# uzh-rpg/event_representation_study

Hardware: AMD Instinct MI355X
Metric: events/sec/GPU (OptimizedRep, Gen1 640x480) + 12-rep GWD matrix wall-time (higher is better)
Workload: dtype f64

## Files before the change

event_representation_study_amd/csrc/evrep_bin.hip:

```cpp
#include "evrep_common.h"

namespace evrep {

#ifndef EVREP_BIN_THREADS
#define EVREP_BIN_THREADS 256
#endif
constexpr int kBinThreads = EVREP_BIN_THREADS;
constexpr int kBinWaves = kBinThreads / kWave;

template <typename Op>
__device__ inline int wave_reduce_dpp(int v, int identity, Op op) {
    v = op(v, __builtin_amdgcn_update_dpp(identity, v, 0x111, 0xf, 0xf, false));
    v = op(v, __builtin_amdgcn_update_dpp(identity, v, 0x112, 0xf, 0xf, false));
    v = op(v, __builtin_amdgcn_update_dpp(identity, v, 0x114, 0xf, 0xf, false));
    v = op(v, __builtin_amdgcn_update_dpp(identity, v, 0x118, 0xf, 0xf, false));
    v = op(v, __builtin_amdgcn_update_dpp(identity, v, 0x142, 0xa, 0xf, false));
    v = op(v, __builtin_amdgcn_update_dpp(identity, v, 0x143, 0xc, 0xf, false));
    return __builtin_amdgcn_readlane(v, 63);
}
__device__ inline int wave_min(int v) { return wave_reduce_dpp(v, INT32_MAX, [](int a, int b) { return min(a, b); }); }
__device__ inline int wave_max(int v) { return wave_reduce_dpp(v, INT32_MIN, [](int a, int b) { return max(a, b); }); }
__device__ inline uint32_t wave_or(uint32_t v) { return (uint32_t)wave_reduce_dpp((int)v, 0, [](int a, int b) { return a | b; }); }
__device__ inline int wave_sum(int v) { return wave_reduce_dpp(v, 0, [](int a, int b) { return a + b; }); }

__device__ inline void wave_phase_lds() {
    __builtin_amdgcn_fence(__ATOMIC_RELEASE, "wavefront");
    __builtin_amdgcn_wave_barrier();
    __builtin_amdgcn_fence(__ATOMIC_ACQUIRE, "wavefront");
}

struct BlockStats {
    int32_t tmin, tmax, xmin, xmax, ymin, ymax;
    uint32_t neg_flags, oob_flags, status;
    int32_t n_valid;
    int32_t pad[2];
};
static_assert(sizeof(BlockStats) == 48, "BlockStats");

__device__ inline void stats_identity(BlockStats &s) {
    s.tmin = INT32_MAX; s.tmax = INT32_MIN; s.xmin = INT32_MAX; s.xmax = INT32_MIN; s.ymin = INT32_MAX; s.ymax = INT32_MIN;
    s.neg_flags = 0; s.oob_flags = 0; s.status = 0; s.n_valid = 0; s.pad[0] = 0; s.pad[1] = 0;
}
__device__ inline void stats_merge(BlockStats &a, const BlockStats &b) {
    a.tmin = min(a.tmin, b.tmin); a.tmax = max(a.tmax, b.tmax);
    a.xmin = min(a.xmin, b.xmin); a.xmax = max(a.xmax, b.xmax);
    a.ymin = min(a.ymin, b.ymin); a.ymax = max(a.ymax, b.ymax);
    a.neg_flags |= b.neg_flags; a.oob_flags |= b.oob_flags; a.status |= b.status; a.n_valid += b.n_valid;
}
__device__ inline void stats_wave_reduce(BlockStats &s) {
    s.tmin = wave_min(s.tmin); s.tmax = wave_max(s.tmax);
    s.xmin = wave_min(s.xmin); s.xmax = wave_max(s.xmax);
    s.ymin = wave_min(s.ymin); s.ymax = wave_max(s.ymax);
    s.neg_flags = wave_or(s.neg_flags); s.oob_flags = wave_or(s.oob_flags); s.status = wave_or(s.status);
    s.n_valid = wave_sum(s.n_valid);
}

constexpr int kRegBatch = 8;

__device__ inline bool decode_window_block(int B, int nblk, int &b, int &blk) {
    const int id = blockIdx.x;
    const int per_group = 8 * nblk;
    const int grp = id / per_group, r = id - grp * per_group;
    const int nw = min(8, B - 8 * grp);
    if (nw == 8) {
        b = grp * 8 + (r & 7);
        blk = r >> 3;
        return true;
    }
    if (r >= nw * nblk) return false;
    b = grp * 8 + r / nblk;
    blk = r - (r / nblk) * nblk;
    return true;
}

#ifdef EVREP_TU_CORE
static __global__ __launch_bounds__(kBinThreads) void k_row_hist(const int4 *__restrict__ ev, const int64_t *__restrict__ off,
                                                      int B, int H, int W, int chunk, int nblk,
                                                      uint32_t *__restrict__ table, BlockStats *__restrict__ stats) {
    extern __shared__ uint32_t hist[];
    __shared__ BlockStats wstats[kBinWaves];
    int b, blk;
    if (!decode_window_block(B, nblk, b, blk)) return;
    const int64_t beg = off[b];
    const int64_t n = off[b + 1] - beg;
    const int64_t lo = (int64_t)blk * chunk;
    if (lo >= n) return;
    for (int i = threadIdx.x; i < H; i += kBinThreads) hist[i] = 0;
    __syncthreads();
    const int64_t hi = (lo + chunk < n) ? lo + chunk : n;
    const MdesWindows mw = mdes_windows(n);
    const int64_t HW = (int64_t)H * W;
    BlockStats st;
    stats_identity(st);
    for (int64_t r0 = lo; r0 < hi; r0 += (int64_t)kRegBatch * kBinThreads) {
        int4 e[kRegBatch];
        int tprev[kRegBatch];
#pragma unroll
        for (int i = 0; i < kRegBatch; ++i) {
            const int64_t r = r0 + (int64_t)i * kBinThreads + threadIdx.x;
            e[i] = make_int4(0, 0, INT32_MAX, 0);
            tprev[i] = INT32_MIN;
            if (r < hi) {
                e[i] = ev[beg + r];
                if ((threadIdx.x & 63) == 0 && r > 0) tprev[i] = ev[beg + r - 1].z;
            }
        }
#pragma unroll
        for (int i = 0; i < kRegBatch; ++i) {
            const int up = __shfl_up(e[i].z, 1, 64);
            if ((threadIdx.x & 63) != 0) tprev[i] = up;
        }
#pragma unroll
        for (int i = 0; i < kRegBatch; ++i) {
            const int64_t r = r0 + (int64_t)i * kBinThreads + threadIdx.x;
            if (r < hi) {
                const int64_t key = (int64_t)e[i].x + (int64_t)e[i].y * W;
                const uint32_t memb = mdes_membership(mw, (int32_t)r);
                if (e[i].w == -1) st.neg_flags |= memb;
                if (key >= 0 && key < HW) {
                    atomicAdd(&hist[(uint32_t)key / (uint32_t)W], 1u);
                    ++st.n_valid;
                } else {
                    st.status |= EVREP_ST_OOB;
                    const int cls = e[i].w == 1 ? 1 : (e[i].w == -1 ? 2 : (e[i].w == 0 ? 3 : 0));
                    st.oob_flags |= memb | (cls ? (memb << (7 * cls)) : 0u);
                }
                if (tprev[i] > e[i].z) st.status |= EVREP_ST_UNSORTED;
                st.tmin = min(st.tmin, e[i].z); st.tmax = max(st.tmax, e[i].z);
                st.xmin = min(st.xmin, e[i].x); st.xmax = max(st.xmax, e[i].x);
                st.ymin = min(st.ymin, e[i].y); st.ymax = max(st.ymax, e[i].y);
            }
        }
    }
    stats_wave_reduce(st);
    if ((threadIdx.x & 63) == 0) wstats[threadIdx.x >> 6] = st;
    __syncthreads();
    if (threadIdx.x == 0) {
        BlockStats t = wstats[0];
        for (int w = 1; w < kBinWaves; ++w) stats_merge(t, wstats[w]);
        stats[(size_t)b * nblk + blk] = t;
    }
    uint32_t *dst = table + ((size_t)b * nblk + blk) * H;
    for (int i = threadIdx.x; i < H; i += kBinThreads) dst[i] = hist[i];
}
#endif

#ifdef EVREP_TU_CORE
static __global__ __launch_bounds__(kBinThreads) void k_row_scan(const int64_t *__restrict__ off, int H, int chunk, int nblk,
                                                      uint32_t *__restrict__ table, uint32_t *__restrict__ row_off,
                                                      const BlockStats *__restrict__ stats, WindowMeta *__restrict__ meta) {
    extern __shared__ uint32_t rowtot[];
    __shared__ BlockStats wstats[kBinWaves];
    __shared__ uint32_t tmp[kBinWaves];
    const int b = blockIdx.x;
    const int64_t beg = off[b];
    const int64_t n = off[b + 1] - beg;
    const int nb = (int)((n + chunk - 1) / chunk);
    BlockStats st;
    stats_identity(st);
    for (int blk = threadIdx.x; blk < nb; blk += kBinThreads) stats_merge(st, stats[(size_t)b * nblk + blk]);
    stats_wave_reduce(st);
    if ((threadIdx.x & 63) == 0) wstats[threadIdx.x >> 6] = st;
    for (int r = threadIdx.x; r < H; r += kBinThreads) {
        uint32_t run = 0;
        for (int b0 = 0; b0 < nb; b0 += kRegBatch) {
            uint32_t v[kRegBatch];
#pragma unroll
            for (int i = 0; i < kRegBatch; ++i)
                v[i] = (b0 + i < nb) ? table[((size_t)b * nblk + b0 + i) * H + r] : 0u;
#pragma unroll
            for (int i = 0; i < kRegBatch; ++i)
                if (b0 + i < nb) { table[((size_t)b * nblk + b0 + i) * H + r] = run; run += v[i]; }
        }
        rowtot[r] = run;
    }
    __syncthreads();
    const int per = (H + kBinThreads - 1) / kBinThreads;
    const int r0 = threadIdx.x * per;
    uint32_t local = 0;
    for (int k = 0; k < per; ++k) if (r0 + k < H) local += rowtot[r0 + k];
    uint32_t total;
    uint32_t run = block_exclusive_scan<kBinWaves>(local, tmp, &total);
    for (int k = 0; k < per; ++k)
        if (r0 + k < H) { const uint32_t t = rowtot[r0 + k]; rowtot[r0 + k] = run; run += t; }
    __syncthreads();
    uint32_t *ro = row_off + (size_t)b * (H + 1);
    for (int r = threadIdx.x; r < H; r += kBinThreads) ro[r] = (uint32_t)beg + rowtot[r];
    if (threadIdx.x == 0) {
        ro[H] = (uint32_t)beg + total;
        BlockStats t = wstats[0];
        for (int w = 1; w < kBinWaves; ++w) stats_merge(t, wstats[w]);
        WindowMeta m;
        m.tmin = t.tmin; m.tmax = t.tmax; m.xmin = t.xmin; m.xmax = t.xmax; m.ymin = t.ymin; m.ymax = t.ymax;
        m.neg_flags = t.neg_flags; m.oob_flags = t.oob_flags; m.status = t.status; m.n_valid = t.n_valid;
        if (n <= 0) m.status |= EVREP_ST_EMPTY;
        else if (t.tmin == t.tmax) m.status |= EVREP_ST_FLAT_TIME;
        for (int i = 0; i < 6; ++i) m.pad[i] = 0;
        meta[b] = m;
    }
}
#endif

#ifdef EVREP_TU_CORE
static __global__ __launch_bounds__(kBinThreads) void k_row_scatter(const int4 *__restrict__ ev, const int64_t *__restrict__ off,
                                                         int B, int H, int W, int chunk, int nblk,
                                                         const uint32_t *__restrict__ table,
                                                         const uint32_t *__restrict__ row_off, Rec *__restrict__ sorted1) {
    extern __shared__ uint32_t cnt[];
    int b, blk;
    if (!decode_window_block(B, nblk, b, blk)) return;
    const int64_t beg = off[b];
    const int64_t n = off[b + 1] - beg;
    const int64_t lo = (int64_t)blk * chunk;
    if (lo >= n) return;
    const int64_t hi = (lo + chunk < n) ? lo + chunk : n;
    const int64_t nloc = hi - lo;
    const int lane = threadIdx.x & 63, wave = threadIdx.x >> 6;
    const int64_t wlo = lo + nloc * wave / kBinWaves, whi = lo + nloc * (wave + 1) / kBinWaves;
    const int64_t HW = (int64_t)H * W;
    constexpr int kSuper = kRegBatch * kWave;
    const int nsuper = (int)((whi - wlo + kSuper - 1) / kSuper);
    for (int i = threadIdx.x; i < kBinWaves * H; i += kBinThreads) cnt[i] = 0;
    __syncthreads();
    uint32_t *mycnt = cnt + wave * H;
    int4 e[kRegBatch];
    for (int sb = 0; sb < nsuper; ++sb) {
#pragma unroll
        for (int i = 0; i < kRegBatch; ++i) {
            const int64_t r = wlo + (int64_t)sb * kSuper + i * kWave + lane;
            e[i] = make_int4(-1, -1, 0, 0);
            if (r < whi) e[i] = ev[beg + r];
        }
#pragma unroll
        for (int i = 0; i < kRegBatch; ++i) {
            const int64_t r = wlo + (int64_t)sb * kSuper + i * kWave + lane;
            const int64_t key = (int64_t)e[i].x + (int64_t)e[i].y * W;
            if (r < whi && key >= 0 && key < HW) atomicAdd(&mycnt[(uint32_t)key / (uint32_t)W], 1u);
        }
    }
    __syncthreads();
    for (int row = threadIdx.x; row < H; row += kBinThreads) {
        uint32_t base = row_off[(size_t)b * (H + 1) + row] + table[((size_t)b * nblk + blk) * H + row];
#pragma unroll
        for (int w = 0; w < kBinWaves; ++w) { const uint32_t t = cnt[w * H + row]; cnt[w * H + row] = base; base += t; }
    }
    __syncthreads();
    const int nbits = bits_for(H);
    volatile uint32_t *vcnt = mycnt;
    for (int sb = 0; sb < nsuper; ++sb) {
        if (nsuper > 1) {
#pragma unroll
            for (int i = 0; i < kRegBatch; ++i) {
                const int64_t r = wlo + (int64_t)sb * kSuper + i * kWave + lane;
                e[i] = make_int4(-1, -1, 0, 0);
                if (r < whi) e[i] = ev[beg + r];
            }
        }
#pragma unroll
        for (int i = 0; i < kRegBatch; ++i) {
            const int64_t r0 = wlo + (int64_t)sb * kSuper + i * kWave;
            if (r0 >= whi) break;
            const int64_t r = r0 + lane;
            const int64_t key = (int64_t)e[i].x + (int64_t)e[i].y * W;
            const bool valid = r < whi && key >= 0 && key < HW;
            const uint32_t row = valid ? (uint32_t)key / (uint32_t)W : 0u;
            uint32_t rk; bool last;
            wave_match(row, nbits, valid, lane, rk, last);
            uint32_t pos = 0;
            if (valid) {
                pos = vcnt[row] + rk;
                sorted1[pos] = make_int4((int)key, (int)r, e[i].z, e[i].w);
            }
            __builtin_amdgcn_wave_barrier();
            if (valid && last) vcnt[row] = pos + 1;
            __builtin_amdgcn_wave_barrier();
        }
    }
}
#endif

constexpr int kStageRecs = 2048;
__host__ __device__ inline size_t fused_scatter_lds_bytes(int H) {
    return (size_t)(kBinWaves + 3) * H * sizeof(uint32_t) + (size_t)kStageRecs * sizeof(Rec);
}

#ifdef EVREP_TU_CORE
static __global__ __launch_bounds__(kBinThreads) void k_row_scatter_fused(const int4 *__restrict__ ev, const int64_t *__restrict__ off,
                                                               int B, int H, int W, int chunk, int nblk,
                                                               const uint32_t *__restrict__ table,
                                                               const BlockStats *__restrict__ stats,
                                                               uint32_t *__restrict__ row_off, WindowMeta *__restrict__ meta,
                                                               Rec *__restrict__ sorted1) {
    extern __shared__ __align__(16) unsigned char smem_raw[];
    Rec *stage = reinterpret_cast<Rec *>(smem_raw);
    uint32_t *cnt = reinterpret_cast<uint32_t *>(stage + kStageRecs);
    uint32_t *rowtot = cnt + kBinWaves * H;
    uint32_t *lbase = rowtot + H;
    uint32_t *delta = lbase + H;
    __shared__ BlockStats wstats[kBinWaves];
    __shared__ uint32_t tmp[kBinWaves];
    int b, blk;
    if (!decode_window_block(B, nblk, b, blk)) return;
    const int64_t beg = off[b];
    const int64_t n = off[b + 1] - beg;
    const int64_t lo = (int64_t)blk * chunk;
    if (lo >= n && !(blk == 0)) return;
    const int nb = (int)((n + chunk - 1) / chunk);
    if (n <= 0) {
        uint32_t *ro = row_off + (size_t)b * (H + 1);
        for (int r = threadIdx.x; r <= H; r += kBinThreads) ro[r] = (uint32_t)beg;
        if (threadIdx.x == 0) {
            WindowMeta m;
            m.tmin = INT32_MAX; m.tmax = INT32_MIN; m.xmin = INT32_MAX; m.xmax = INT32_MIN; m.ymin = INT32_MAX; m.ymax = INT32_MIN;
            m.neg_flags = 0; m.oob_flags = 0; m.status = EVREP_ST_EMPTY; m.n_valid = 0;
            for (int i = 0; i < 6; ++i) m.pad[i] = 0;
            meta[b] = m;
        }
        return;
    }
    const int64_t hi = (lo + chunk < n) ? lo + chunk : n;
    const int64_t nloc = hi - lo;
    const int lane = threadIdx.x & 63, wave = threadIdx.x >> 6;
    const int64_t wlo = lo + nloc * wave / kBinWaves, whi = lo + nloc * (wave + 1) / kBinWaves;
    const int64_t HW = (int64_t)H * W;
    for (int i = threadIdx.x; i < kBinWaves * H; i += kBinThreads) cnt[i] = 0;
    __syncthreads();
    uint32_t *mycnt = cnt + wave * H;
    int4 e[kRegBatch];
#pragma unroll
    for (int i = 0; i < kRegBatch; ++i) {
        const int64_t r = wlo + i * kWave + lane;
        e[i] = make_int4(-1, -1, 0, 0);
        if (r < whi) e[i] = ev[beg + r];
    }
#pragma unroll
    for (int i = 0; i < kRegBatch; ++i) {
        const int64_t r = wlo + i * kWave + lane;
        const int64_t key = (int64_t)e[i].x + (int64_t)e[i].y * W;
        if (r < whi && key >= 0 && key < HW) atomicAdd(&mycnt[(uint32_t)key / (uint32_t)W], 1u);
    }
    if (blk == 0) {
        BlockStats st;
        stats_identity(st);
        for (int k = threadIdx.x; k < nb; k += kBinThreads) stats_merge(st, stats[(size_t)b * nblk + k]);
        stats_wave_reduce(st);
        if (lane == 0) wstats[wave] = st;
    }
    __syncthreads();
    for (int r = threadIdx.x; r < H; r += kBinThreads) {
        uint32_t tot = 0, before = 0;
        for (int b0 = 0; b0 < nb; b0 += kRegBatch) {
            uint32_t v[kRegBatch];
#pragma unroll
            for (int i = 0; i < kRegBatch; ++i) v[i] = (b0 + i < nb) ? table[((size_t)b * nblk + b0 + i) * H + r] : 0u;
#pragma unroll
            for (int i = 0; i < kRegBatch; ++i) { tot += v[i]; if (b0 + i < blk) before += v[i]; }
        }
        rowtot[r] = tot;
        delta[r] = before;
        uint32_t own = 0;
#pragma unroll
        for (int w = 0; w < kBinWaves; ++w) own += cnt[w * H + r];
        lbase[r] = own;
    }
    __syncthreads();
    const int per = (H + kBinThreads - 1) / kBinThreads;
    const int r0 = threadIdx.x * per;
    uint32_t loc_t = 0, loc_o = 0;
    for (int k = 0; k < per; ++k) if (r0 + k < H) { loc_t += rowtot[r0 + k]; loc_o += lbase[r0 + k]; }
    uint32_t total_t, total_o;
    uint32_t run_t = block_exclusive_scan<kBinWaves>(loc_t, tmp, &total_t);
    uint32_t run_o = block_exclusive_scan<kBinWaves>(loc_o, tmp, &total_o);
    for (int k = 0; k < per; ++k)
        if (r0 + k < H) {
            const uint32_t t = rowtot[r0 + k]; rowtot[r0 + k] = run_t; run_t += t;
            const uint32_t o = lbase[r0 + k];  lbase[r0 + k] = run_o;  run_o += o;
        }
    __syncthreads();
    for (int r = threadIdx.x; r < H; r += kBinThreads) {
        const uint32_t gstart = (uint32_t)beg + rowtot[r] + delta[r];
        uint32_t base = lbase[r];
        delta[r] = gstart - base;
#pragma unroll
        for (int w = 0; w < kBinWaves; ++w) { const uint32_t t = cnt[w * H + r]; cnt[w * H + r] = base; base += t; }
        if (blk == 0) row_off[(size_t)b * (H + 1) + r] = (uint32_t)beg + rowtot[r];
    }
    if (blk == 0 && threadIdx.x == 0) {
        row_off[(size_t)b * (H + 1) + H] = (uint32_t)beg + total_t;
        BlockStats t = wstats[0];
        for (int w = 1; w < kBinWaves; ++w) stats_merge(t, wstats[w]);
        WindowMeta m;
        m.tmin = t.tmin; m.tmax = t.tmax; m.xmin = t.xmin; m.xmax = t.xmax; m.ymin = t.ymin; m.ymax = t.ymax;
        m.neg_flags = t.neg_flags; m.oob_flags = t.oob_flags; m.status = t.status; m.n_valid = t.n_valid;
        if (t.tmin == t.tmax) m.status |= EVREP_ST_FLAT_TIME;
        for (int i = 0; i < 6; ++i) m.pad[i] = 0;
        meta[b] = m;
    }
    __syncthreads();
    const int nbits = bits_for(H);
    volatile uint32_t *vcnt = mycnt;
#pragma unroll
    for (int i = 0; i < kRegBatch; ++i) {
        const int64_t rr0 = wlo + i * kWave;
        if (rr0 >= whi) break;
        const int64_t r = rr0 + lane;
        const int64_t key = (int64_t)e[i].x + (int64_t)e[i].y * W;
        const bool valid = r < whi && key >= 0 && key < HW;
        const uint32_t row = valid ? (uint32_t)key / (uint32_t)W : 0u;
        uint32_t rk; bool last;
        wave_match(row, nbits, valid, lane, rk, last);
        uint32_t pos = 0;
        if (valid) {
            pos = vcnt[row] + rk;
            stage[pos] = make_int4((int)key, (int)r, e[i].z, e[i].w);
        }
        __builtin_amdgcn_wave_barrier();
        if (valid && last) vcnt[row] = pos + 1;
        __builtin_amdgcn_wave_barrier();
    }
    __syncthreads();
    for (uint32_t t = threadIdx.x; t < total_o; t += kBinThreads) {
        const Rec rec = stage[t];
        const uint32_t row = (uint32_t)rec.x / (uint32_t)W;
        sorted1[delta[row] + t] = rec;
    }
}
#endif

#ifdef EVREP_TU_CORE
static __global__ __launch_bounds__(kWave) void k_col_sort(const Rec *__restrict__ sorted1, const uint32_t *__restrict__ row_off,
                                                   int H, int W, int nchunk, Rec *__restrict__ sorted2,
                                                   uint32_t *__restrict__ chunk_off) {
    extern __shared__ uint32_t cnt[];
    const int b = blockIdx.y, row = blockIdx.x;
    const int lane = threadIdx.x;
    const uint32_t rs = row_off[(size_t)b * (H + 1) + row], re = row_off[(size_t)b * (H + 1) + row + 1];
    const uint32_t n = re - rs;
    uint32_t *co = chunk_off + ((size_t)b * H + row) * (nchunk + 1);
    if (n == 0) {
        for (int c = lane; c <= nchunk; c += kWave) co[c] = rs;
        return;
    }
    constexpr uint32_t kSuper = 4 * kWave;
    const int rowbase = row * W;
    const uint32_t nsuper = (n + kSuper - 1) / kSuper;
    Rec e[4];
    for (int i = lane; i < W; i += kWave) cnt[i] = 0;
    __syncthreads();
    for (uint32_t sb = 0; sb < nsuper; ++sb) {
#pragma unroll
        for (int i = 0; i < 4; ++i) {
            const uint32_t j = sb * kSuper + i * kWave + lane;
            e[i] = make_int4(0, 0, 0, 0);
            if (j < n) e[i] = sorted1[rs + j];
        }
#pragma unroll
        for (int i = 0; i < 4; ++i)
            if (sb * kSuper + i * kWave + lane < n) atomicAdd(&cnt[e[i].x - rowbase], 1u);
    }
    __syncthreads();
    const int per = (W + kWave - 1) / kWave;
    const int c0 = lane * per;
    uint32_t local = 0;
    for (int k = 0; k < per; ++k) if (c0 + k < W) local += cnt[c0 + k];
    uint32_t incl = local;
#pragma unroll
    for (int d = 1; d < 64; d <<= 1) { const uint32_t o = __shfl_up(incl, d, 64); if (lane >= d) incl += o; }
    uint32_t run = incl - local;
    for (int k = 0; k < per; ++k)
        if (c0 + k < W) { const uint32_t t = cnt[c0 + k]; cnt[c0 + k] = run; run += t; }
    __syncthreads();
    for (int c = lane; c <= nchunk; c += kWave) co[c] = (c * kChunkPx < W) ? rs + cnt[c * kChunkPx] : re;
    __syncthreads();
    const int nbits = bits_for(W);
    volatile uint32_t *vcnt = cnt;
    for (uint32_t sb = 0; sb < nsuper; ++sb) {
        if (nsuper > 1) {
#pragma unroll
            for (int i = 0; i < 4; ++i) {
                const uint32_t j = sb * kSuper + i * kWave + lane;
                e[i] = make_int4(0, 0, 0, 0);
                if (j < n) e[i] = sorted1[rs + j];
            }
        }
#pragma unroll
        for (int i = 0; i < 4; ++i) {
            const uint32_t j0 = sb * kSuper + i * kWave;
            if (j0 >= n) break;
            const bool valid = j0 + lane < n;
            const uint32_t col = valid ? (uint32_t)(e[i].x - rowbase) : 0u;
            uint32_t rk; bool last;
            wave_match(col, nbits, valid, lane, rk, last);
            uint32_t pos = 0;
            if (valid) {
                pos = vcnt[col] + rk;
                sorted2[rs + pos] = e[i];
            }
            __builtin_amdgcn_wave_barrier();
            if (valid && last) vcnt[col] = pos + 1;
            __builtin_amdgcn_wave_barrier();
        }
    }
}
#endif

#ifndef BS_DEBUG
#define BS_DEBUG 0
#endif
constexpr int kBsThreads = 1024;
constexpr int kBsWaves = kBsThreads / kWave;
constexpr int kBsPerLane = 8;
constexpr int kBsChunk = kBsThreads * kBsPerLane;
constexpr int kBsMaxBlocks = 64;
constexpr int kBsChainBlocks = 16;

__host__ __device__ inline int bs_hp(int H) { return (H + 1) & ~1; }
__host__ __device__ inline size_t block_rowsort_lds_bytes(int H) {
    return (size_t)kBsChunk * sizeof(Rec) + (size_t)kBsWaves * bs_hp(H) * sizeof(uint16_t) + (size_t)(H + 2) * sizeof(uint32_t);
}

#ifdef EVREP_TU_CORE
static __global__ __launch_bounds__(kBsThreads) void k_block_rowsort(const int4 *__restrict__ ev, const int64_t *__restrict__ off,
                                                             int B, int H, int W, int nblk, uint32_t *__restrict__ table,
                                                             BlockStats *__restrict__ stats, Rec *__restrict__ sorted1) {
    extern __shared__ __align__(16) unsigned char smem_raw[];
    Rec *stage = reinterpret_cast<Rec *>(smem_raw);
    const int Hp = bs_hp(H), Hw = Hp >> 1;
    uint16_t *cnt16 = reinterpret_cast<uint16_t *>(stage + kBsChunk);
    uint32_t *cnt32 = reinterpret_cast<uint32_t *>(cnt16);
    uint32_t *lbase = reinterpret_cast<uint32_t *>(cnt16 + (size_t)kBsWaves * Hp);
    __shared__ BlockStats wstats[kBsWaves];
    __shared__ uint32_t tmp[kBsWaves];
    int b, blk;
    if (!decode_window_block(B, nblk, b, blk)) return;
    const int64_t beg = off[b];
    const int64_t n = off[b + 1] - beg;
    const int64_t lo = (int64_t)blk * kBsChunk;
    if (lo >= n) return;
    const int64_t hi = (lo + kBsChunk < n) ? lo + kBsChunk : n;
    const int lane = threadIdx.x & 63, wave = threadIdx.x >> 6;
    const int64_t wlo = lo + (int64_t)wave * (kBsPerLane * kWave);
    const int64_t whi = (wlo + kBsPerLane * kWave < hi) ? wlo + kBsPerLane * kWave : hi;
    const int64_t HW = (int64_t)H * W;
    int4 e[kBsPerLane];
    int tprev[kBsPerLane];
#pragma unroll
    for (int i = 0; i < kBsPerLane; ++i) {
        const int64_t r = wlo + i * kWave + lane;
        e[i] = make_int4(-1, -1, INT32_MAX, 0);
        tprev[i] = INT32_MIN;
        if (r < whi) {
            e[i] = ev[beg + r];
            if (lane == 0 && r > 0) tprev[i] = ev[beg + r - 1].z;
        }
    }
    for (int i = threadIdx.x; i < kBsWaves * Hw; i += kBsThreads) cnt32[i] = 0;
    __syncthreads();
    const MdesWindows mw = mdes_windows(n);
    uint32_t full = 0, part = 0;
#pragma unroll
    for (int i = 0; i < 7; ++i) {
        if (mw.lo[i] <= lo && hi <= mw.hi[i]) full |= 1u << i;
        else if (!(hi <= mw.lo[i] || lo >= mw.hi[i])) part |= 1u << i;
    }
    uint32_t *mycnt32 = cnt32 + wave * Hw;
    BlockStats st;
    stats_identity(st);
    uint32_t rows[kBsPerLane];
    uint32_t sneg = 0;
    bool cut = false;
    if (part) {
        const int32_t a0 = (int32_t)wlo, a1 = (int32_t)whi;
#pragma unroll
        for (int q = 0; q < 7; ++q) cut |= (mw.lo[q] > a0 && mw.lo[q] < a1) || (mw.hi[q] > a0 && mw.hi[q] < a1);
    }
    const uint32_t memb_u = cut ? 0u : (full | (part ? (mdes_membership(mw, (int32_t)wlo) & part) : 0u));
#pragma unroll
    for (int i = 0; i < kBsPerLane; ++i) {
        const int64_t r0 = wlo + i * kWave;
        const int64_t r = r0 + lane;
        const bool in = r < whi;
        const int up = __builtin_amdgcn_update_dpp(0, e[i].z, 0x138 , 0xf, 0xf, false);
        if (lane != 0) tprev[i] = up;

        uint32_t row = (uint32_t)e[i].y;
        bool valid = in && (uint32_t)e[i].x < (uint32_t)W && (uint32_t)e[i].y < (uint32_t)H;
        if (__any(in && (uint32_t)e[i].x >= (uint32_t)W)) {
            const int64_t key = (int64_t)e[i].x + (int64_t)e[i].y * W;
            valid = in && key >= 0 && key < HW;
            if (valid) row = (uint32_t)key / (uint32_t)W;
        }
        rows[i] = valid ? row : 0xffffffffu;
        if (valid && !(BS_DEBUG & 8)) atomicAdd(&mycnt32[row >> 1], 1u << ((row & 1u) * 16));
        if (!(BS_DEBUG & 1)) {
            if (!cut) {
                if (__any(in && e[i].w == -1)) sneg |= memb_u;
            } else if (in && e[i].w == -1) {
                st.neg_flags |= full | (mdes_membership(mw, (int32_t)r) & part);
            }
            if (__any(in && !valid)) {
                if (in && !valid) {
                    const uint32_t memb = cut ? (full | (mdes_membership(mw, (int32_t)r) & part)) : memb_u;
                    st.status |= EVREP_ST_OOB;
                    const int cls = e[i].w == 1 ? 1 : (e[i].w == -1 ? 2 : (e[i].w == 0 ? 3 : 0));
                    st.oob_flags |= memb | (cls ? (memb << (7 * cls)) : 0u);
                }
            }
        }
        if (in && !(BS_DEBUG & 1)) {
            if (valid) ++st.n_valid;
            if (tprev[i] > e[i].z) st.status |= EVREP_ST_UNSORTED;
            if ((uint32_t)(e[i].w + 1) > 2u) st.status |= kStEscaped;
            st.tmin = min(st.tmin, e[i].z); st.tmax = max(st.tmax, e[i].z);
            st.xmin = min(st.xmin, e[i].x); st.xmax = max(st.xmax, e[i].x);
            st.ymin = min(st.ymin, e[i].y); st.ymax = max(st.ymax, e[i].y);
        }
    }
    st.neg_flags |= sneg;
    stats_wave_reduce(st);
    if (lane == 0) wstats[wave] = st;
    __syncthreads();
    uint32_t run = 0;
    if ((int)threadIdx.x < Hw) {
#pragma unroll
        for (int w = 0; w < kBsWaves; ++w) { const uint32_t c = cnt32[w * Hw + threadIdx.x]; cnt32[w * Hw + threadIdx.x] = run; run += c; }
    }
    const uint32_t own0 = run & 0xffffu, own1 = run >> 16;
    uint32_t total;
    const uint32_t ex = block_exclusive_scan<kBsWaves>(own0 + own1, tmp, &total);
    if ((int)threadIdx.x < Hw) {
        const uint32_t l0 = ex, l1 = ex + own0;
        const uint32_t add = l0 | (l1 << 16);
#pragma unroll
        for (int w = 0; w < kBsWaves; ++w) cnt32[w * Hw + threadIdx.x] += add;
        uint32_t *tb = table + ((size_t)b * nblk + blk) * (H + 1);
        const int r0 = 2 * (int)threadIdx.x;
        tb[r0] = l0; lbase[r0] = l0;
        if (r0 + 1 < H) { tb[r0 + 1] = l1; lbase[r0 + 1] = l1; }
    }
    if (threadIdx.x == 0) {
        table[((size_t)b * nblk + blk) * (H + 1) + H] = total;
        BlockStats t = wstats[0];
        for (int w = 1; w < kBsWaves; ++w) stats_merge(t, wstats[w]);
        stats[(size_t)b * nblk + blk] = t;
    }
    __syncthreads();
    const int nbits = bits_for(H);
    volatile uint16_t *vpos = cnt16 + (size_t)wave * Hp;
#pragma unroll
    for (int i = 0; i < kBsPerLane; ++i) {
        if (wlo + i * kWave >= whi) break;
        const bool valid = rows[i] != 0xffffffffu;
        const uint32_t row = valid ? rows[i] : 0u;
        uint32_t rk = 0; bool last = false;
        if (!(BS_DEBUG & 2)) wave_match(row, nbits, valid, lane, rk, last);
        uint32_t pos = 0;
        if (valid) {
            pos = (BS_DEBUG & 2) ? (uint32_t)(wave * 512 + i * 64 + lane) : (uint32_t)vpos[row] + rk;
            const int64_t r = wlo + i * kWave + lane;
            const Rec rec = make_int4((int)((int64_t)e[i].x + (int64_t)e[i].y * W), (int)r, e[i].z, e[i].w);
            if (BS_DEBUG & 16) sorted1[beg + lo + pos] = rec; else stage[pos] = rec;
        }
        __builtin_amdgcn_wave_barrier();
        if (valid && last) vpos[row] = (uint16_t)(pos + 1);
        __builtin_amdgcn_wave_barrier();
    }
    __syncthreads();
    Rec *dst = sorted1 + beg + lo;
    if (!(BS_DEBUG & (4 | 16)))
        for (uint32_t t = threadIdx.x; t < total; t += kBsThreads) dst[t] = stage[t];
}
#endif

#ifndef EVREP_CS_WAVES
#define EVREP_CS_WAVES 8
#endif
constexpr int kCsWaves = EVREP_CS_WAVES;
constexpr int kCsRowWaves = 4;
constexpr int kCsMaxRuns = 128;
__host__ __device__ inline int col_sort_per4(int W) { return ((W + kWave - 1) / kWave + 3) / 4; }
__host__ __device__ inline int col_sort_words(int W) { return kWave * 4 * col_sort_per4(W); }
__host__ __device__ inline int col_sort_wave_words(int W) { return col_sort_words(W) + 2 * kCsMaxRuns; }

#ifndef CS_WAVES
#define CS_WAVES 8
#endif
#ifdef EVREP_TU_CORE
static __global__ __launch_bounds__(kCsWaves * kWave) __attribute__((amdgpu_waves_per_eu(CS_WAVES))) void k_col_sort_runs(const int4 *__restrict__ ev, const Rec *__restrict__ sorted1, const int64_t *__restrict__ off,
                                                                     const uint32_t *__restrict__ table,
                                                                     const BlockStats *__restrict__ stats, int H, int W, int nblk,
                                                                     int nchunk, int kpr, int chunk_shift, int by_key,
                                                                     Rec *__restrict__ sorted2,
                                                                     uint32_t *__restrict__ chunk_off, WindowMeta *__restrict__ meta) {
    extern __shared__ __align__(16) uint32_t cnt_all[];
    const int lane = threadIdx.x & 63, wave = threadIdx.x >> 6;
    const int b = blockIdx.y, unit = blockIdx.x * (int)(blockDim.x >> 6) + wave;
    if (unit >= (by_key ? H * kpr : H)) return;
    const int row = by_key ? unit / kpr : unit;
    const int ck = by_key ? unit - row * kpr : 0;
    const int Wu = by_key ? min(kChunkPx, W - ck * kChunkPx) : W;
    uint32_t *cnt = cnt_all + (size_t)wave * col_sort_wave_words(by_key ? kChunkPx : W);
    const int64_t beg = off[b];
    const int64_t n_win = off[b + 1] - beg;
    const int nb = min((int)(((uint32_t)n_win + (1u << chunk_shift) - 1u) >> chunk_shift), nblk);
    uint32_t ta[2] = {0u, 0u}, tb[2] = {0u, 0u};
#pragma unroll
    for (int h = 0; h < 2; ++h) {
        const int k = lane + h * kWave;
        if (k < nb) {
            const uint32_t *tk = table + ((size_t)b * nblk + k) * ((size_t)H * kpr + 1);
            ta[h] = tk[by_key ? (size_t)unit : (size_t)row * kpr];
            tb[h] = tk[by_key ? (size_t)unit + 1 : (size_t)(row + 1) * kpr];
        }
    }
    if (unit == 0) {
        BlockStats st;
        stats_identity(st);
#pragma unroll
        for (int h = 0; h < 2; ++h) {
            const int k = lane + h * kWave;
            if (k < nb) {
                const int4 *sp = reinterpret_cast<const int4 *>(stats + (size_t)b * nblk + k);
                const int4 q0 = sp[0], q1 = sp[1], q2 = sp[2];
                st.tmin = min(st.tmin, q0.x); st.tmax = max(st.tmax, q0.y); st.xmin = min(st.xmin, q0.z); st.xmax = max(st.xmax, q0.w);
                st.ymin = min(st.ymin, q1.x); st.ymax = max(st.ymax, q1.y);
                st.neg_flags |= (uint32_t)q1.z; st.oob_flags |= (uint32_t)q1.w;
                st.status |= (uint32_t)q2.x; st.n_valid += q2.y;
            }
        }
        stats_wave_reduce(st);
        if (lane == 0) {
            WindowMeta m;
            m.tmin = st.tmin; m.tmax = st.tmax; m.xmin = st.xmin; m.xmax = st.xmax; m.ymin = st.ymin; m.ymax = st.ymax;
            m.neg_flags = st.neg_flags; m.oob_flags = st.oob_flags; m.status = st.status & 0xffffu; m.n_valid = st.n_valid;
            if (n_win <= 0) m.status |= EVREP_ST_EMPTY;
            else if (st.tmin == st.tmax) m.status |= EVREP_ST_FLAT_TIME;
            for (int i = 0; i < 6; ++i) m.pad[i] = 0;
            meta[b] = m;
        }
    }
    constexpr uint32_t kSuper = 4 * kWave;
    const uint32_t rbeg = (uint32_t)beg + (uint32_t)wave_sum((int)(ta[0] + ta[1]));
    const uint32_t len0 = tb[0] - ta[0], len1 = tb[1] - ta[1];
    uint32_t incl0 = len0, incl1 = len1;
#pragma unroll
    for (int d = 1; d < 64; d <<= 1) {
        const uint32_t o0 = __shfl_up(incl0, d, 64), o1 = __shfl_up(incl1, d, 64);
        if (lane >= d) { incl0 += o0; incl1 += o1; }
    }
    const uint32_t tot0 = (uint32_t)__builtin_amdgcn_readlane((int)incl0, 63);
    incl1 += tot0;
    const uint32_t n = (uint32_t)__builtin_amdgcn_readlane((int)incl1, 63);
    const uint32_t pre0 = incl0 - len0, pre1 = incl1 - len1;
    const uint32_t src0 = (uint32_t)beg + ((uint32_t)lane << chunk_shift) + ta[0] - pre0;
    const uint32_t src1 = (uint32_t)beg + ((uint32_t)(lane + kWave) << chunk_shift) + ta[1] - pre1;
    const uint32_t rend = rbeg + n;
    uint32_t *runs = cnt + col_sort_words(by_key ? kChunkPx : W);
    if (nb > kBsChainBlocks) {
        runs[lane] = pre0;
        runs[kWave + lane] = pre1;
        runs[kCsMaxRuns + lane] = src0;
        runs[kCsMaxRuns + kWave + lane] = src1;
        wave_phase_lds();
    }
    const Rec8 *sorted8 = reinterpret_cast<const Rec8 *>(sorted1);
    const int4 *evw = ev + beg;
    auto load = [&](uint32_t at) -> Rec {
        return by_key ? rec8_unpack(sorted8[at], row * W, ck * kChunkPx, evw) : sorted1[at];
    };
    auto fetch = [&](uint32_t j) -> Rec {
        if (nb <= kBsChainBlocks) {
            uint32_t s = (uint32_t)__builtin_amdgcn_readlane((int)src0, 0);
            uint32_t prev = s;
            for (int k = 1; k < nb; ++k) {
                const uint32_t pk = (uint32_t)__builtin_amdgcn_readlane((int)pre0, k);
                const uint32_t sk = (uint32_t)__builtin_amdgcn_readlane((int)src0, k);
                s += (j >= pk) ? sk - prev : 0u;
                prev = sk;
            }
            return load(s + j);
        }
        uint32_t lo = 0, hi = (uint32_t)nb;
#pragma unroll
        for (int step = 0; step < 7; ++step) {
            const uint32_t mid = (lo + hi) >> 1;
            const bool go = hi - lo > 1 && runs[mid] <= j;
            if (hi - lo > 1) { if (go) lo = mid; else hi = mid; }
        }
        return load(runs[kCsMaxRuns + lo] + j);
    };
    Rec e[4];
#pragma unroll
    for (int i = 0; i < 4; ++i) {
        const uint32_t j = i * kWave + lane;
        e[i] = make_int4(0, 0, 0, 0);
        if (j < n) e[i] = fetch(j);
    }
    const int nbits = bits_for(Wu);
    const int per4 = col_sort_per4(Wu);
    uint4 *cnt4 = reinterpret_cast<uint4 *>(cnt) + (size_t)lane * per4;
    volatile uint32_t *vcnt = cnt;
    uint32_t *co = chunk_off + ((size_t)b * H + row) * (nchunk + 1);
    if (by_key && lane == 0) {
        co[ck] = rbeg;
        if (ck == kpr - 1) co[kpr] = rend;
    }
    if (n == 0) {
        if (!by_key) for (int c = lane; c <= nchunk; c += kWave) co[c] = rbeg;
        return;
    }
    const int rowbase = row * W + ck * kChunkPx;
    const uint32_t nsuper = (n + kSuper - 1) / kSuper;
    for (int k = 0; k < per4; ++k) cnt4[k] = make_uint4(0u, 0u, 0u, 0u);
    wave_phase_lds();
#pragma unroll
    for (int i = 0; i < 4; ++i)
        if ((uint32_t)(i * kWave + lane) < n) atomicAdd(&cnt[e[i].x - rowbase], 1u);
    for (uint32_t sb = 1; sb < nsuper; ++sb)
        for (int i = 0; i < 4; ++i) {
            const uint32_t j = sb * kSuper + i * kWave + lane;
            if (j < n) atomicAdd(&cnt[fetch(j).x - rowbase], 1u);
        }
    wave_phase_lds();
    uint32_t local = 0;
    for (int k = 0; k < per4; ++k) { const uint4 v = cnt4[k]; local += v.x + v.y + v.z + v.w; }
    uint32_t inc2 = local;
#pragma unroll
    for (int d = 1; d < 64; d <<= 1) { const uint32_t o = __shfl_up(inc2, d, 64); if (lane >= d) inc2 += o; }
    uint32_t run = inc2 - local;
    for (int k = 0; k < per4; ++k) {
        const uint4 v = cnt4[k];
        uint4 o;
        o.x = run; o.y = o.x + v.x; o.z = o.y + v.y; o.w = o.z + v.z;
        run = o.w + v.w;
        cnt4[k] = o;
    }
    wave_phase_lds();
    if (!by_key) for (int c = lane; c <= nchunk; c += kWave) co[c] = (c * kChunkPx < W) ? rbeg + cnt[c * kChunkPx] : rend;
    wave_phase_lds();
    for (uint32_t sb = 0; sb < nsuper; ++sb) {
#pragma unroll
        for (int i = 0; i < 4; ++i) {
            const uint32_t j0 = sb * kSuper + i * kWave;
            if (j0 >= n) break;
            const bool valid = j0 + lane < n;
            Rec rec = e[i];
            if (sb > 0) { rec = make_int4(0, 0, 0, 0); if (valid) rec = fetch(j0 + lane); }
            const uint32_t col = valid ? (uint32_t)(rec.x - rowbase) : 0u;
            uint32_t rk; bool last;
            wave_match(col, nbits, valid, lane, rk, last);
            uint32_t pos = 0;
            if (valid) {
                pos = vcnt[col] + rk;
                sorted2[rbeg + pos] = rec;
            }
            __builtin_amdgcn_wave_barrier();
            if (valid && last) vcnt[col] = pos + 1;
            __builtin_amdgcn_wave_barrier();
        }
    }
}
#endif

#ifndef KS_DIRECT_WRITE
#define KS_DIRECT_WRITE 0
#endif
#ifndef KS_DEBUG
#define KS_DEBUG 0
#endif
constexpr int kKsHotGroup = 16;
__host__ __device__ inline size_t block_keysort_lds_bytes(int NK, int cap, int chunk) {
    return (size_t)cap * sizeof(Rec8) + (size_t)chunk * sizeof(uint16_t) + (size_t)(NK + 4) * sizeof(uint32_t);
}

#ifndef KS_WAVES_512
#define KS_WAVES_512 6
#endif
#ifndef KS_WAVES_1024
#define KS_WAVES_1024 8
#endif
template <int TPB, int PL = 8>
__global__ __launch_bounds__(TPB) __attribute__((amdgpu_waves_per_eu(TPB == 1024 ? KS_WAVES_1024 : KS_WAVES_512))) void k_block_keysort(const int4 *__restrict__ ev, const int64_t *__restrict__ off,
                                                             int B, int H, int W, int kpr, int nblk, int cap,
                                                             uint32_t *__restrict__ table, BlockStats *__restrict__ stats,
                                                             Rec *__restrict__ sorted1, int64_t *__restrict__ nwin,
                                                             uint32_t *__restrict__ hot) {
    extern __shared__ __align__(16) unsigned char smem_raw[];
    constexpr int kChunk = TPB * PL, kNW = TPB / kWave, kPerWave = PL * kWave;
    if (blockIdx.x == 0 && threadIdx.x < 128) hot[threadIdx.x * 16] = 0u;
    const int NK = H * kpr;
    Rec8 *stage = reinterpret_cast<Rec8 *>(smem_raw);
    uint16_t *rankbuf = reinterpret_cast<uint16_t *>(stage + cap);
    uint32_t *base = reinterpret_cast<uint32_t *>(rankbuf + kChunk);
    __shared__ int bstats[12];
    __shared__ uint32_t tmp[kNW];
    __shared__ uint32_t nhot_s;
    int b, blk;
    if (!decode_window_block(B, nblk, b, blk)) return;
    const int64_t beg = off[b];
    const int64_t n = off[b + 1] - beg;
    const int64_t lo = (int64_t)blk * kChunk;
    if (blk == 0 && threadIdx.x == 0) nwin[b] = n;
    if (lo >= n) return;
    const int nblock = (int)((lo + kChunk < n) ? kChunk : n - lo);
    const int lane = threadIdx.x & 63, wave = threadIdx.x >> 6;
    const int w0 = wave * kPerWave;
    const int lo32 = (int)lo;
    const int4 *evb = ev + beg + lo;
    int4 e[PL];
    int tprev[PL];
#pragma unroll
    for (int i = 0; i < PL; ++i) {
        const int li = w0 + i * kWave + lane;
        e[i] = make_int4(-1, -1, INT32_MAX, 0);
        tprev[i] = INT32_MIN;
        if (li < nblock) {
            e[i] = evb[li];
            if (lane == 0 && (li > 0 || lo > 0)) tprev[i] = evb[li - 1].z;
        }
    }
    for (int i = threadIdx.x; i <= NK; i += TPB) base[i] = 0;
    if (threadIdx.x == 0) nhot_s = 0u;
    if (threadIdx.x < 12) {
        const int f = threadIdx.x;
        bstats[f] = (f == 0 || f == 2 || f == 4) ? INT32_MAX : ((f == 1 || f == 3 || f == 5) ? INT32_MIN : 0);
    }
    __syncthreads();
    const MdesWindows mw = mdes_windows(n);
    uint32_t full = 0, part = 0;
#pragma unroll
    for (int i = 0; i < 7; ++i) {
        if (mw.lo[i] <= lo32 && lo32 + nblock <= mw.hi[i]) full |= 1u << i;
        else if (!(lo32 + nblock <= mw.lo[i] || lo32 >= mw.hi[i])) part |= 1u << i;
    }
    BlockStats st;
    stats_identity(st);
    uint32_t ko[PL];
    uint32_t sneg = 0;
    bool cut = false;
    const int a0 = lo32 + w0, a1 = min(lo32 + w0 + kPerWave, lo32 + nblock);
    if (part) {
#pragma unroll
        for (int q = 0; q < 7; ++q) cut |= (mw.lo[q] > a0 && mw.lo[q] < a1) || (mw.hi[q] > a0 && mw.hi[q] < a1);
    }
    const uint32_t memb_u = cut ? 0u : (full | (part ? (mdes_membership(mw, a0) & part) : 0u));
    const int HW = H * W;
#pragma unroll
    for (int i = 0; i < PL; ++i) {
        const int li = w0 + i * kWave + lane;
        const bool in = li < nblock;
        const int up = __builtin_amdgcn_update_dpp(0, e[i].z, 0x138 , 0xf, 0xf, false);
        if (lane != 0) tprev[i] = up;
        uint32_t row = (uint32_t)e[i].y, col = (uint32_t)e[i].x;
        bool valid = in && (uint32_t)e[i].x < (uint32_t)W && (uint32_t)e[i].y < (uint32_t)H;
        if (__any(in && (uint32_t)e[i].x >= (uint32_t)W)) {
            const int64_t key = (int64_t)e[i].x + (int64_t)e[i].y * W;
            valid = in && key >= 0 && key < (int64_t)HW;
            if (valid) { row = (uint32_t)key / (uint32_t)W; col = (uint32_t)key - row * (uint32_t)W; }
        }
        ko[i] = 0xffffffffu;
        if (valid) {
            const uint32_t key = row * (uint32_t)kpr + (col >> 7);
            ko[i] = key | (atomicAdd(&base[key], 1u) << 16);
        }
        if (KS_DEBUG & 4) continue;
        if (!cut) {
            if (__any(in && e[i].w == -1)) sneg |= memb_u;
        } else if (in && e[i].w == -1) {
            st.neg_flags |= full | (mdes_membership(mw, lo32 + li) & part);
        }
        if (__any(in && !valid)) {
            if (in && !valid) {
                const uint32_t memb = cut ? (full | (mdes_membership(mw, lo32 + li) & part)) : memb_u;
                st.status |= EVREP_ST_OOB;
                const int cls = e[i].w == 1 ? 1 : (e[i].w == -1 ? 2 : (e[i].w == 0 ? 3 : 0));
                st.oob_flags |= memb | (cls ? (memb << (7 * cls)) : 0u);
            }
        }
        if (in) {
            if (valid) ++st.n_valid;
            if (tprev[i] > e[i].z) st.status |= EVREP_ST_UNSORTED;
            if ((uint32_t)(e[i].w + 1) > 2u) st.status |= kStEscaped;
            st.tmin = min(st.tmin, e[i].z); st.tmax = max(st.tmax, e[i].z);
            st.xmin = min(st.xmin, e[i].x); st.xmax = max(st.xmax, e[i].x);
            st.ymin = min(st.ymin, e[i].y); st.ymax = max(st.ymax, e[i].y);
        }
    }
    st.neg_flags |= sneg;
    stats_wave_reduce(st);
    if (lane == 0) {
        atomicMin(&bstats[0], st.tmin); atomicMax(&bstats[1], st.tmax);
        atomicMin(&bstats[2], st.xmin); atomicMax(&bstats[3], st.xmax);
        atomicMin(&bstats[4], st.ymin); atomicMax(&bstats[5], st.ymax);
        atomicOr(reinterpret_cast<uint32_t *>(&bstats[6]), st.neg_flags);
        atomicOr(reinterpret_cast<uint32_t *>(&bstats[7]), st.oob_flags);
        atomicOr(reinterpret_cast<uint32_t *>(&bstats[8]), st.status);
        atomicAdd(&bstats[9], st.n_valid);
    }
    __syncthreads();
    const int per = (NK + TPB - 1) / TPB;
    const int k0 = (int)threadIdx.x * per;
    uint32_t local = 0;
    for (int k = 0; k < per; ++k) if (k0 + k < NK) local += base[k0 + k];
    uint32_t total;
    uint32_t run = block_exclusive_scan<kNW>(local, tmp, &total);
    for (int k = 0; k < per; ++k)
        if (k0 + k < NK) {
            const uint32_t c = base[k0 + k];
            uint32_t tag = 0u;
            if (c > (uint32_t)kKsHotGroup) tag = (atomicAdd(&nhot_s, 1u) + 1u) << 16;
            base[k0 + k] = run | tag;
            run += c;
        }
    if (threadIdx.x == 0) base[NK] = total;
    if (threadIdx.x < 12) reinterpret_cast<int *>(stats + (size_t)b * nblk + blk)[threadIdx.x] = bstats[threadIdx.x];
    __syncthreads();
    uint32_t *tb = table + ((size_t)b * nblk + blk) * ((size_t)NK + 1);
    if (!(KS_DEBUG & 8))
        for (int k = threadIdx.x; k <= NK; k += TPB) tb[k] = base[k] & 0xffffu;
    const uint32_t nhot = nhot_s;
    const uint32_t mine0 = (uint32_t)(w0 + lane);
#pragma unroll
    for (int i = 0; i < PL; ++i) {
        if (ko[i] != 0xffffffffu) {
            const uint32_t bw = base[ko[i] & 0xffffu];
            if (!(bw >> 16)) rankbuf[(bw & 0xffffu) + (ko[i] >> 16)] = (uint16_t)(mine0 + i * kWave);
        }
    }
    if (nhot) {
        constexpr int kHs = kChunk / 16;
        uint32_t *hcnt = reinterpret_cast<uint32_t *>(stage);
        for (uint32_t t = lane; t < nhot; t += kWave) hcnt[wave * kHs + t] = 0u;
        wave_phase_lds();
#pragma unroll
        for (int i = 0; i < PL; ++i)
            if (ko[i] != 0xffffffffu) {
                const uint32_t hsl = base[ko[i] & 0xffffu] >> 16;
                if (hsl) atomicAdd(&hcnt[wave * kHs + hsl - 1u], 1u);
            }
        __syncthreads();
        if (threadIdx.x < nhot) {
            uint32_t acc = 0;
            for (int w = 0; w < kNW; ++w) { const uint32_t c = hcnt[w * kHs + threadIdx.x]; hcnt[w * kHs + threadIdx.x] = acc; acc += c; }
        }
        __syncthreads();
        const int hbits = bits_for((int)nhot);
        volatile uint32_t *vh = hcnt + wave * kHs;
#pragma unroll
        for (int i = 0; i < PL; ++i) {
            const uint32_t bw = ko[i] != 0xffffffffu ? base[ko[i] & 0xffffu] : 0u;
            const bool hot = (bw >> 16) != 0u;
            if (!__any(hot)) continue;
            const uint32_t slot = hot ? (bw >> 16) - 1u : 0u;
            uint32_t rk; bool last;
            wave_match(slot, hbits, hot, lane, rk, last);
            uint32_t pos = 0;
            if (hot) {
                pos = vh[slot] + rk;
                ko[i] = ((bw & 0xffffu) + pos) | 0x80000000u;
            }
            __builtin_amdgcn_wave_barrier();
            if (hot && last) vh[slot] = pos + 1;
            __builtin_amdgcn_wave_barrier();
        }
    }
    __syncthreads();
    {
        uint32_t gb[PL], g[PL], sm[PL];
        uint32_t gmax = 0;
#pragma unroll
        for (int i = 0; i < PL; ++i) {
            gb[i] = 0; g[i] = 0; sm[i] = 0;
            if (ko[i] != 0xffffffffu && !(ko[i] >> 31)) {
                const uint32_t key = ko[i] & 0xffffu;
                const uint32_t bw = base[key];
                gb[i] = bw & 0xffffu;
                g[i] = (bw >> 16) ? 0u : (base[key + 1] & 0xffffu) - gb[i];
                if (KS_DEBUG & 1) { sm[i] = ko[i] >> 16; g[i] = 0; }
                if (g[i] == 1) g[i] = 0;
                gmax = max(gmax, g[i]);
            }
        }
        gmax = (uint32_t)wave_max((int)gmax);
        for (uint32_t j = 0; j < gmax; ++j) {
#pragma unroll
            for (int i = 0; i < PL; ++i)
                if (j < g[i]) sm[i] += (uint32_t)rankbuf[gb[i] + j] < mine0 + (uint32_t)(i * kWave) ? 1u : 0u;
        }
#pragma unroll
        for (int i = 0; i < PL; ++i)
            if (ko[i] != 0xffffffffu) ko[i] = (ko[i] >> 31) ? (ko[i] & 0x7fffffffu) : gb[i] + sm[i];
    }
    if (nhot) __syncthreads();
    Rec8 *dst = reinterpret_cast<Rec8 *>(sorted1) + beg + lo;
#if KS_DIRECT_WRITE
#pragma unroll
    for (int i = 0; i < PL; ++i) {
        if (ko[i] != 0xffffffffu && !(KS_DEBUG & 2)) {
            int col = e[i].x;
            if ((uint32_t)col >= (uint32_t)W) { const uint32_t key = (uint32_t)(e[i].x + e[i].y * W); col = (int)(key % (uint32_t)W); }
            dst[ko[i]] = rec8_pack(col, lo32 + w0 + i * kWave + lane, e[i].z, e[i].w);
        }
    }
    return;
#endif
    for (uint32_t pb = 0; pb < total && !(KS_DEBUG & 2); pb += (uint32_t)cap) {
        if (pb) __syncthreads();
#pragma unroll
        for (int i = 0; i < PL; ++i) {
            const uint32_t pos = ko[i] - pb;
            if (pos < (uint32_t)cap) {
                int col = e[i].x;
                if ((uint32_t)col >= (uint32_t)W) { const uint32_t key = (uint32_t)(e[i].x + e[i].y * W); col = (int)(key % (uint32_t)W); }
                stage[pos] = rec8_pack(col, lo32 + w0 + i * kWave + lane, e[i].z, e[i].w);
            }
        }
        __syncthreads();
        const uint32_t cnt = min((uint32_t)cap, total - pb);
        for (uint32_t t = threadIdx.x; t < cnt; t += TPB) dst[pb + t] = stage[t];
    }
}

#ifdef EVREP_TU_CORE
static __global__ __launch_bounds__(kWave) void k_window_meta(const int64_t *__restrict__ nwin, const BlockStats *__restrict__ stats,
                                                      int nblk, int chunk_shift, WindowMeta *__restrict__ meta) {
    const int b = blockIdx.x, lane = threadIdx.x;
    const int64_t n_win = nwin[b];
    const int nb = min((int)(((uint32_t)n_win + (1u << chunk_shift) - 1u) >> chunk_shift), nblk);
    BlockStats st;
    stats_identity(st);
    for (int k = lane; k < nb; k += kWave) stats_merge(st, stats[(size_t)b * nblk + k]);
    stats_wave_reduce(st);
    if (lane == 0) {
        WindowMeta m;
        m.tmin = st.tmin; m.tmax = st.tmax; m.xmin = st.xmin; m.xmax = st.xmax; m.ymin = st.ymin; m.ymax = st.ymax;
        m.neg_flags = st.neg_flags; m.oob_flags = st.oob_flags; m.status = st.status & 0xffffu; m.n_valid = st.n_valid;
        if (n_win <= 0) m.status |= EVREP_ST_EMPTY;
        else if (st.tmin == st.tmax) m.status |= EVREP_ST_FLAT_TIME;
        for (int i = 0; i < 6; ++i) m.pad[i] = 0;
        meta[b] = m;
    }
}
#endif

}
```

Baseline: 9.215 billion.

## Restructure key-sort binning: defer stats, clamp loads, vectorize writeback and scan

Loads events with clamped indices and carries a single previous timestamp per wave instead of one per slot. The per-event stats and membership work moves into a lambda that, for small PL, runs after the scatter/writeback, taking it off the path to the first barrier. Other changes: the LDS histogram is zeroed with 16-byte stores, the block scan becomes an inline shuffle scan, the wrap check is hoisted into one wave vote, and the staged output is written as paired 16-byte stores. This adds code complexity and register pressure, and the deferred stats add another barrier at the end.

```diff
diff --git a/event_representation_study_amd/csrc/evrep_bin.hip b/event_representation_study_amd/csrc/evrep_bin.hip
--- a/event_representation_study_amd/csrc/evrep_bin.hip
+++ b/event_representation_study_amd/csrc/evrep_bin.hip
@@ -908,52 +908,104 @@
     const int lo32 = (int)lo;
     const int4 *evb = ev + beg + lo;
     int4 e[PL];
-    int tprev[PL];
-#pragma unroll
-    for (int i = 0; i < PL; ++i) {
-        const int li = w0 + i * kWave + lane;
-        e[i] = make_int4(-1, -1, INT32_MAX, 0);
-        tprev[i] = INT32_MIN;
-        if (li < nblock) {
-            e[i] = evb[li];
-            if (lane == 0 && (li > 0 || lo > 0)) tprev[i] = evb[li - 1].z;
-        }
-    }
-    for (int i = threadIdx.x; i <= NK; i += TPB) base[i] = 0;
+#pragma unroll
+    for (int i = 0; i < PL; ++i) e[i] = evb[min(w0 + i * kWave + lane, nblock - 1)];
+    const bool has_prev = w0 < nblock && (w0 > 0 || lo > 0);
+    int tprev0 = evb[has_prev ? w0 - 1 : 0].z;
+    if (!has_prev) tprev0 = INT32_MIN;
+#pragma unroll
+    for (int i = 0; i < PL; ++i)
+        if (w0 + i * kWave + lane >= nblock) e[i] = make_int4(-1, -1, INT32_MAX, 0);
+    for (int i = threadIdx.x; i <= NK / 4; i += TPB) reinterpret_cast<uint4 *>(base)[i] = make_uint4(0u, 0u, 0u, 0u);
     if (threadIdx.x == 0) nhot_s = 0u;
     if (threadIdx.x < 12) {
         const int f = threadIdx.x;
         bstats[f] = (f == 0 || f == 2 || f == 4) ? INT32_MAX : ((f == 1 || f == 3 || f == 5) ? INT32_MIN : 0);
     }
     __syncthreads();
-    const MdesWindows mw = mdes_windows(n);
-    uint32_t full = 0, part = 0;
-#pragma unroll
-    for (int i = 0; i < 7; ++i) {
-        if (mw.lo[i] <= lo32 && lo32 + nblock <= mw.hi[i]) full |= 1u << i;
-        else if (!(lo32 + nblock <= mw.lo[i] || lo32 >= mw.hi[i])) part |= 1u << i;
-    }
-    BlockStats st;
-    stats_identity(st);
+    constexpr bool kStatsLast = PL <= 4;
     uint32_t ko[PL];
-    uint32_t sneg = 0;
-    bool cut = false;
-    const int a0 = lo32 + w0, a1 = min(lo32 + w0 + kPerWave, lo32 + nblock);
-    if (part) {
-#pragma unroll
-        for (int q = 0; q < 7; ++q) cut |= (mw.lo[q] > a0 && mw.lo[q] < a1) || (mw.hi[q] > a0 && mw.hi[q] < a1);
-    }
-    const uint32_t memb_u = cut ? 0u : (full | (part ? (mdes_membership(mw, a0) & part) : 0u));
+    uint32_t vmask = 0;
+    auto block_stats = [&]() {
+        BlockStats st;
+        stats_identity(st);
+        if (!(KS_DEBUG & 4)) {
+            const MdesWindows mw = mdes_windows(n);
+            uint32_t full = 0, part = 0;
+#pragma unroll
+            for (int i = 0; i < 7; ++i) {
+                if (mw.lo[i] <= lo32 && lo32 + nblock <= mw.hi[i]) full |= 1u << i;
+                else if (!(lo32 + nblock <= mw.lo[i] || lo32 >= mw.hi[i])) part |= 1u << i;
+            }
+            bool cut = false;
+            const int a0 = lo32 + w0, a1 = min(lo32 + w0 + kPerWave, lo32 + nblock);
+            if (part) {
+#pragma unroll
+                for (int q = 0; q < 7; ++q) cut |= (mw.lo[q] > a0 && mw.lo[q] < a1) || (mw.hi[q] > a0 && mw.hi[q] < a1);
+            }
+            const uint32_t memb_u = cut ? 0u : (full | (part ? (mdes_membership(mw, a0) & part) : 0u));
+            bool neg = false, oob = false;
+#pragma unroll
+            for (int i = 0; i < PL; ++i) {
+                const int li = w0 + i * kWave + lane;
+                const bool in = li < nblock, valid = (vmask >> i) & 1u;
+                int tprev = __builtin_amdgcn_update_dpp(0, e[i].z, 0x138 , 0xf, 0xf, false);
+                if (lane == 0) tprev = i == 0 ? tprev0 : __builtin_amdgcn_readlane(e[i > 0 ? i - 1 : 0].z, 63);
+                neg |= in && e[i].w == -1;
+                oob |= in && !valid;
+                if (in) {
+                    if (valid) ++st.n_valid;
+                    if (tprev > e[i].z) st.status |= EVREP_ST_UNSORTED;
+                    if ((uint32_t)(e[i].w + 1) > 2u) st.status |= kStEscaped;
+                    st.tmin = min(st.tmin, e[i].z); st.tmax = max(st.tmax, e[i].z);
+                    st.xmin = min(st.xmin, e[i].x); st.xmax = max(st.xmax, e[i].x);
+                    st.ymin = min(st.ymin, e[i].y); st.ymax = max(st.ymax, e[i].y);
+                }
+            }
+            if (!cut) {
+                if (__any(neg)) st.neg_flags |= memb_u;
+            } else if (neg) {
+#pragma unroll
+                for (int i = 0; i < PL; ++i) {
+                    const int li = w0 + i * kWave + lane;
+                    if (li < nblock && e[i].w == -1) st.neg_flags |= full | (mdes_membership(mw, lo32 + li) & part);
+                }
+            }
+            if (__any(oob)) {
+#pragma unroll
+                for (int i = 0; i < PL; ++i) {
+                    const int li = w0 + i * kWave + lane;
+                    if (li < nblock && !((vmask >> i) & 1u)) {
+                        const uint32_t memb = cut ? (full | (mdes_membership(mw, lo32 + li) & part)) : memb_u;
+                        st.status |= EVREP_ST_OOB;
+                        const int cls = e[i].w == 1 ? 1 : (e[i].w == -1 ? 2 : (e[i].w == 0 ? 3 : 0));
+                        st.oob_flags |= memb | (cls ? (memb << (7 * cls)) : 0u);
+                    }
+                }
+            }
+        }
+        stats_wave_reduce(st);
+        if (lane == 0) {
+            atomicMin(&bstats[0], st.tmin); atomicMax(&bstats[1], st.tmax);
+            atomicMin(&bstats[2], st.xmin); atomicMax(&bstats[3], st.xmax);
+            atomicMin(&bstats[4], st.ymin); atomicMax(&bstats[5], st.ymax);
+            atomicOr(reinterpret_cast<uint32_t *>(&bstats[6]), st.neg_flags);
+            atomicOr(reinterpret_cast<uint32_t *>(&bstats[7]), st.oob_flags);
+            atomicOr(reinterpret_cast<uint32_t *>(&bstats[8]), st.status);
+            atomicAdd(&bstats[9], st.n_valid);
+        }
+    };
     const int HW = H * W;
+    bool wraps = false;
+#pragma unroll
+    for (int i = 0; i < PL; ++i) wraps |= w0 + i * kWave + lane < nblock && (uint32_t)e[i].x >= (uint32_t)W;
+    const bool any_wrap = __any(wraps);
 #pragma unroll
     for (int i = 0; i < PL; ++i) {
-        const int li = w0 + i * kWave + lane;
-        const bool in = li < nblock;
-        const int up = __builtin_amdgcn_update_dpp(0, e[i].z, 0x138 , 0xf, 0xf, false);
-        if (lane != 0) tprev[i] = up;
+        const bool in = w0 + i * kWave + lane < nblock;
         uint32_t row = (uint32_t)e[i].y, col = (uint32_t)e[i].x;
         bool valid = in && (uint32_t)e[i].x < (uint32_t)W && (uint32_t)e[i].y < (uint32_t)H;
-        if (__any(in && (uint32_t)e[i].x >= (uint32_t)W)) {
+        if (any_wrap) {
             const int64_t key = (int64_t)e[i].x + (int64_t)e[i].y * W;
             valid = in && key >= 0 && key < (int64_t)HW;
             if (valid) { row = (uint32_t)key / (uint32_t)W; col = (uint32_t)key - row * (uint32_t)W; }
@@ -962,48 +1014,27 @@
         if (valid) {
             const uint32_t key = row * (uint32_t)kpr + (col >> 7);
             ko[i] = key | (atomicAdd(&base[key], 1u) << 16);
-        }
-        if (KS_DEBUG & 4) continue;
-        if (!cut) {
-            if (__any(in && e[i].w == -1)) sneg |= memb_u;
-        } else if (in && e[i].w == -1) {
-            st.neg_flags |= full | (mdes_membership(mw, lo32 + li) & part);
-        }
-        if (__any(in && !valid)) {
-            if (in && !valid) {
-                const uint32_t memb = cut ? (full | (mdes_membership(mw, lo32 + li) & part)) : memb_u;
-                st.status |= EVREP_ST_OOB;
-                const int cls = e[i].w == 1 ? 1 : (e[i].w == -1 ? 2 : (e[i].w == 0 ? 3 : 0));
-                st.oob_flags |= memb | (cls ? (memb << (7 * cls)) : 0u);
-            }
-        }
-        if (in) {
-            if (valid) ++st.n_valid;
-            if (tprev[i] > e[i].z) st.status |= EVREP_ST_UNSORTED;
-            if ((uint32_t)(e[i].w + 1) > 2u) st.status |= kStEscaped;
-            st.tmin = min(st.tmin, e[i].z); st.tmax = max(st.tmax, e[i].z);
-            st.xmin = min(st.xmin, e[i].x); st.xmax = max(st.xmax, e[i].x);
-            st.ymin = min(st.ymin, e[i].y); st.ymax = max(st.ymax, e[i].y);
-        }
-    }
-    st.neg_flags |= sneg;
-    stats_wave_reduce(st);
-    if (lane == 0) {
-        atomicMin(&bstats[0], st.tmin); atomicMax(&bstats[1], st.tmax);
-        atomicMin(&bstats[2], st.xmin); atomicMax(&bstats[3], st.xmax);
-        atomicMin(&bstats[4], st.ymin); atomicMax(&bstats[5], st.ymax);
-        atomicOr(reinterpret_cast<uint32_t *>(&bstats[6]), st.neg_flags);
-        atomicOr(reinterpret_cast<uint32_t *>(&bstats[7]), st.oob_flags);
-        atomicOr(reinterpret_cast<uint32_t *>(&bstats[8]), st.status);
-        atomicAdd(&bstats[9], st.n_valid);
-    }
+            vmask |= 1u << i;
+        }
+    }
+    if (!kStatsLast) block_stats();
     __syncthreads();
     const int per = (NK + TPB - 1) / TPB;
     const int k0 = (int)threadIdx.x * per;
     uint32_t local = 0;
     for (int k = 0; k < per; ++k) if (k0 + k < NK) local += base[k0 + k];
-    uint32_t total;
-    uint32_t run = block_exclusive_scan<kNW>(local, tmp, &total);
+    uint32_t total = 0, run;
+    {
+        uint32_t incl = local;
+#pragma unroll
+        for (int d = 1; d < 64; d <<= 1) { const uint32_t o = __shfl_up(incl, d, 64); if (lane >= d) incl += o; }
+        if (lane == 63) tmp[wave] = incl;
+        __syncthreads();
+        uint32_t wbase = 0;
+#pragma unroll
+        for (int w = 0; w < kNW; ++w) { const uint32_t t = tmp[w]; if (w < wave) wbase += t; total += t; }
+        run = wbase + incl - local;
+    }
     for (int k = 0; k < per; ++k)
         if (k0 + k < NK) {
             const uint32_t c = base[k0 + k];
@@ -1013,7 +1044,7 @@
             run += c;
         }
     if (threadIdx.x == 0) base[NK] = total;
-    if (threadIdx.x < 12) reinterpret_cast<int *>(stats + (size_t)b * nblk + blk)[threadIdx.x] = bstats[threadIdx.x];
+    if (!kStatsLast && threadIdx.x < 12) reinterpret_cast<int *>(stats + (size_t)b * nblk + blk)[threadIdx.x] = bstats[threadIdx.x];
     __syncthreads();
     uint32_t *tb = table + ((size_t)b * nblk + blk) * ((size_t)NK + 1);
     if (!(KS_DEBUG & 8))
@@ -1102,8 +1133,8 @@
             dst[ko[i]] = rec8_pack(col, lo32 + w0 + i * kWave + lane, e[i].z, e[i].w);
         }
     }
-    return;
-#endif
+#else
+    const int odd = (int)((uint32_t)(beg + lo) & 1u);
     for (uint32_t pb = 0; pb < total && !(KS_DEBUG & 2); pb += (uint32_t)cap) {
         if (pb) __syncthreads();
 #pragma unroll
@@ -1116,8 +1147,22 @@
             }
         }
         __syncthreads();
-        const uint32_t cnt = min((uint32_t)cap, total - pb);
-        for (uint32_t t = threadIdx.x; t < cnt; t += TPB) dst[pb + t] = stage[t];
+        const int cnt = (int)min((uint32_t)cap, total - pb);
+        for (int t = 2 * (int)threadIdx.x - odd; t < cnt; t += 2 * TPB) {
+            if (t >= 0 && t + 1 < cnt) {
+                const Rec8 r0 = stage[t], r1 = stage[t + 1];
+                gstore16(dst + pb + t, make_uint4(r0.x, r0.y, r1.x, r1.y));
+            } else {
+                const int t1 = t < 0 ? 0 : t;
+                dst[pb + t1] = stage[t1];
+            }
+        }
+    }
+#endif
+    if (kStatsLast) {
+        block_stats();
+        __syncthreads();
+        if (threadIdx.x < 12) reinterpret_cast<int *>(stats + (size_t)b * nblk + blk)[threadIdx.x] = bstats[threadIdx.x];
     }
 }
 
```

Result: no change. 9.149 billion (-0.7%).
